# IuvenisSapiens/Qwen3-TTS-Rust

Measured on AMD Instinct MI355X. Metric: audio-seconds generated per second (aggregate over GPUs) = concurrent real-time streams; RTF and first-chunk latency from the single-utterance leg, higher is better.
Workload: dtype i8

## Files before the change

### qwen3-tts-rust_amd/csrc/kernels.hip

```cpp
#include "kernels.h"
#include <cstdlib>
#include "q3_common.h"
#include "../../include/q3tts_spec.h"
#include "kdev.h"
#include "wslice.h"

namespace q3 {

Q3_STAMP_SETTER(set_stamp_buffer)

template <int LPR, int MT>
__global__ void __launch_bounds__(512) k_gemv_q8(Q8Mat w, int row0, int nrows, const int8_t* __restrict__ xq,
                                                 const uint16_t* __restrict__ xd, float* __restrict__ out,
                                                 int out_stride, int ntok) {
    constexpr int R = 64 / LPR, BPL = LPR / 2, NLD = 8 / BPL;
    __shared__ float red[8][R * MT];
    const int lane = threadIdx.x & 63, wave = threadIdx.x >> 6;
    const int r = lane % R, q = lane / R, half = q & 1, bil = q >> 1;
    const int nseg = w.K >> 8, nb = w.K >> 5;
    const int sseg = blockIdx.y, seg = sseg * 8 + wave;
    const int tok0 = blockIdx.z * MT;
    const bool active = seg < nseg;
    float acc[MT];
#pragma unroll
    for (int m = 0; m < MT; m++) acc[m] = 0.0f;
    if (active) {
        int row = row0 + blockIdx.x * R + r;
        if (row > w.Npad - 1) row = w.Npad - 1;
        const int rg = row >> 5, r32 = row & 31;
        const uint8_t* base = w.qs + ((size_t)rg * nb + (size_t)seg * 8) * 1024 + half * 512 + r32 * 16;
        uint4 wv[NLD];
#pragma unroll
        for (int i = 0; i < NLD; i++) wv[i] = *reinterpret_cast<const uint4*>(base + (size_t)(i * BPL + bil) * 1024);
        const uint4 dwv = *reinterpret_cast<const uint4*>(w.sc + (((size_t)rg * nseg + seg) * 32 + r32) * 8);
#pragma unroll
        for (int m = 0; m < MT; m++) {
            int tok = tok0 + m;
            if (tok > ntok - 1) tok = ntok - 1;
            const int8_t* xp = xq + (size_t)tok * w.K + seg * 256;
            const uint4 dxv = *reinterpret_cast<const uint4*>(xd + (size_t)tok * nb + seg * 8);
#pragma unroll
            for (int i = 0; i < NLD; i++) {
                const uint4 xv = *reinterpret_cast<const uint4*>(xp + (i * BPL + bil) * 32 + half * 16);
                int isum = dot16(wv[i], xv);
                isum += xor_lane<R>(isum);
#pragma unroll
                for (int j = 0; j < BPL; j++) {
                    const int isj = (BPL == 1) ? isum : __shfl(isum, r + 2 * j * R);
                    const int b = i * BPL + j;
                    const float sc = h2f(half_of(dwv, b)) * h2f(half_of(dxv, b));
                    acc[m] = q3_fmaf((float)isj, sc, acc[m]);
                }
            }
        }
        if (q == 0) {
#pragma unroll
            for (int m = 0; m < MT; m++) red[wave][m * R + r] = acc[m];
        }
    }
    wg_barrier_lds();
    for (int t = threadIdx.x; t < R * MT; t += blockDim.x) {
        const int m = t / R, rr = t % R;
        int nsg = nseg - sseg * 8;
        if (nsg > 8) nsg = 8;
        float v[8];
#pragma unroll
        for (int s = 0; s < 8; s++) v[s] = red[s][t];
        float S = v[0];
#pragma unroll
        for (int s = 1; s < 8; s++) S = (s < nsg) ? S + v[s] : S;
        const int orow = blockIdx.x * R + rr, tok = tok0 + m;
        if (orow < nrows && tok < ntok) out[((size_t)sseg * ntok + tok) * out_stride + orow] = S;
    }
}

__global__ void k_gemm_q8_tok(Q8Mat w, int row0, int nrows, const int8_t* __restrict__ xq, const uint16_t* __restrict__ xd,
                              float* __restrict__ out, int out_stride, int ntok);
#define Q3_GEMM_Q8_BUDGET __launch_bounds__(512) __attribute__((amdgpu_waves_per_eu(4, 4)))
template <bool GU>
__global__ void Q3_GEMM_Q8_BUDGET k_gemm_q8_mfma(Q8Mat w, int row0, int nrows, const int8_t* __restrict__ xq, const uint16_t* __restrict__ xd,
                               float* __restrict__ out, int out_stride, int ntok, int ff, int8_t* __restrict__ aq, uint16_t* __restrict__ ad);
template <bool GU>
__global__ void Q3_GEMM_Q8_BUDGET k_gemm_q8_tile1(Q8Mat w, int row0, int nrows, const int8_t* __restrict__ xq, const uint16_t* __restrict__ xd,
                               float* __restrict__ out, int out_stride, int ntok, int ff, int8_t* __restrict__ aq, uint16_t* __restrict__ ad);
#define Q3_GEMM_Q8_WIDE_BUDGET __launch_bounds__(256) __attribute__((amdgpu_waves_per_eu(2, 2)))
template <bool GU>
__global__ void Q3_GEMM_Q8_WIDE_BUDGET k_gemm_q8_wide(Q8Mat w, int row0, int nrows, const int8_t* __restrict__ xq, const uint16_t* __restrict__ xd,
// ... 865 lines not shown
                        const int orow = blockIdx.x * 32 + rr;
                        if (orow < nrows && tok < ntok) out[((size_t)sseg * ntok + tok) * out_stride + orow] = S;
                    } else if (q == 0) gate_s[lt][t] = S;
                    else {
                        const float y = q3_swiglu(gate_s[lt][t], S);
                        float amax = q3_fabsf(y);
                        amax = fmaxf(amax, xor_lane<16>(amax)); amax = fmaxf(amax, xor_lane<8>(amax)); amax = fmaxf(amax, xor_lane<4>(amax));
                        amax = fmaxf(amax, xor_lane<2>(amax)); amax = fmaxf(amax, xor_lane<1>(amax));
                        const float dd = amax / 127.0f;
                        const float id = (dd != 0.0f) ? (1.0f / dd) : 0.0f;
                        if (tok < ntok) {
                            aq[(size_t)tok * ff + blockIdx.x * 32 + rr] = (int8_t)(int)q3_rintf(y * id);
                            if (rr == 0) ad[(size_t)tok * (ff >> 5) + blockIdx.x] = f2h(dd);
                        }
                    }
                }
                wg_barrier_lds();
            }
        }
    });
}


__global__ void __launch_bounds__(64) k_rmsnorm_quant(NormArgs a) {
    const int tok = blockIdx.x, lane = threadIdx.x;
    const int nch = a.d >> 8;
    const float* hin = a.h_in;
    if (a.idx_keys) hin += (size_t)key_code(a.idx_keys[(size_t)tok * a.idx_stride]) * a.h_stride;
    else if (a.idx) hin += (size_t)a.idx[(size_t)tok * a.idx_stride] * a.h_stride;
    else hin += (size_t)tok * a.h_stride;
    float4 x[8];
    float p = 0.0f;
#pragma unroll
    for (int c = 0; c < 8; c++) {
        if (c < nch) {
            float4 v = *reinterpret_cast<const float4*>(hin + 256 * c + 4 * lane);
            if (a.nparts > 0) {
                const float* pp = a.parts + (size_t)tok * a.parts_stride + 256 * c + 4 * lane;
                float4 y = *reinterpret_cast<const float4*>(pp);
                for (int s = 1; s < a.nparts; s++) {
                    const float4 z = *reinterpret_cast<const float4*>(pp + (size_t)s * gridDim.x * a.parts_stride);
                    y.x = y.x + z.x; y.y = y.y + z.y; y.z = y.z + z.z; y.w = y.w + z.w;
                }
                v.x = v.x + y.x; v.y = v.y + y.y; v.z = v.z + y.z; v.w = v.w + y.w;
            }
            if (a.h_out) *reinterpret_cast<float4*>(a.h_out + (size_t)tok * a.d + 256 * c + 4 * lane) = v;
            x[c] = v;
            p = q3_fmaf(v.x, v.x, p); p = q3_fmaf(v.y, v.y, p); p = q3_fmaf(v.z, v.z, p); p = q3_fmaf(v.w, v.w, p);
        }
    }
    const float ss = wave_sum_bfly(p);
    const float mean = ss / (float)a.d;
    const float scale = 1.0f / q3_sqrtf(mean + a.eps);
#pragma unroll
    for (int c = 0; c < 8; c++) {
        if (c < nch) {
            const float4 g = *reinterpret_cast<const float4*>(a.g + 256 * c + 4 * lane);
            float4 y;
            y.x = (x[c].x * scale) * g.x; y.y = (x[c].y * scale) * g.y;
            y.z = (x[c].z * scale) * g.z; y.w = (x[c].w * scale) * g.w;
            if (a.xn_out) *reinterpret_cast<float4*>(a.xn_out + (size_t)tok * a.d + 256 * c + 4 * lane) = y;
            float amax = fmaxf(fmaxf(q3_fabsf(y.x), q3_fabsf(y.y)), fmaxf(q3_fabsf(y.z), q3_fabsf(y.w)));
            amax = fmaxf(amax, xor_lane<1>(amax)); amax = fmaxf(amax, xor_lane<2>(amax)); amax = fmaxf(amax, xor_lane<4>(amax));
            const float dd = amax / 127.0f;
            const float id = (dd != 0.0f) ? (1.0f / dd) : 0.0f;
            const int q0 = (int)q3_rintf(y.x * id), q1 = (int)q3_rintf(y.y * id), q2 = (int)q3_rintf(y.z * id), q3v = (int)q3_rintf(y.w * id);
            const uint32_t pk = (uint32_t)(q0 & 0xFF) | ((uint32_t)(q1 & 0xFF) << 8) | ((uint32_t)(q2 & 0xFF) << 16) | ((uint32_t)(q3v & 0xFF) << 24);
            *reinterpret_cast<uint32_t*>(a.xq + (size_t)tok * a.d + 256 * c + 4 * lane) = pk;
            if ((lane & 7) == 0) a.xd[(size_t)tok * (a.d >> 5) + 8 * c + (lane >> 3)] = f2h(dd);
        }
    }
}
void launch_rmsnorm_quant(hipStream_t st, const NormArgs& a, int ntok) {
    hipLaunchKernelGGL(k_rmsnorm_quant, dim3(ntok), dim3(64), 0, st, a);
}

__global__ void __launch_bounds__(64) k_qk_rope_append(QkvRows qkv, int n_head, int n_kv,
                                                       const float* __restrict__ q_norm_w, const float* __restrict__ k_norm_w,
                                                       float eps, const float* __restrict__ rope_cos,
                                                       const float* __restrict__ rope_sin, int n_ctx,
                                                       const int32_t* __restrict__ mrope_sec, TokMeta tm, KvCache kv,
                                                       int layer, float* __restrict__ qrot) {
    const int hv = blockIdx.x, tok = blockIdx.y, lane = threadIdx.x;
    const float* vec = qkv.row(tok) + (size_t)hv * 128;
    float x1 = vec[lane], x2 = vec[lane + 64];
    const int seq = tm.seq_of(tok), slot = tm.slot_of(tok);
    const int page = kv.page_of(seq, slot >> 6);
    const int ps = slot & 63;
    if (hv < n_head + n_kv) {
        const float* w = hv < n_head ? q_norm_w : k_norm_w;
        float p = x1 * x1;
        p = q3_fmaf(x2, x2, p);
        const float ss = wave_sum_bfly(p);
        const float mean = ss / 128.0f;
        const float scale = 1.0f / q3_sqrtf(mean + eps);
        const float y1 = (x1 * scale) * w[lane], y2 = (x2 * scale) * w[lane + 64];
        int32_t sec[4] = { mrope_sec[0], mrope_sec[1], mrope_sec[2], mrope_sec[3] };
        int pp = tm.pos_of(tok, q3_mrope_stream(lane, sec));
        if (pp < 0) pp = 0;
        if (pp > n_ctx - 1) pp = n_ctx - 1;
        float o1, o2;
        q3_rope_pair(y1, y2, rope_cos[(size_t)pp * 64 + lane], rope_sin[(size_t)pp * 64 + lane], &o1, &o2);
        if (hv < n_head) {
            float* dst = qrot + ((size_t)tok * n_head + hv) * 128;
            dst[lane] = o1; dst[lane + 64] = o2;
        } else {
            const int kh = hv - n_head;
            uint16_t* Kb = kv.k + (size_t)page * kv.page_stride() + (size_t)layer * kv.layer_stride() + (size_t)kh * 8192;
            Kb[((lane >> 3) * 64 + ps) * 8 + (lane & 7)] = f2h(o1);
            Kb[(((lane + 64) >> 3) * 64 + ps) * 8 + (lane & 7)] = f2h(o2);
        }
    } else {
        const int vh = hv - n_head - n_kv;
        uint16_t* Vb = kv.v + (size_t)page * kv.page_stride() + (size_t)layer * kv.layer_stride() + (size_t)vh * 8192;
        Vb[ps * 128 + lane] = f2h(x1);
        Vb[ps * 128 + lane + 64] = f2h(x2);
    }
}
void launch_qk_rope_append(hipStream_t st, const QkvRows& qkv, const float*, int n_head, int n_kv,
                           const float* q_norm_w, const float* k_norm_w, float eps, const float* rope_cos,
                           const float* rope_sin, int n_ctx, const int32_t* mrope_sec, const TokMeta& tm,
                           const KvCache& kv, int layer, float* qrot, int ntok) {
    hipLaunchKernelGGL(k_qk_rope_append, dim3(n_head + 2 * n_kv, ntok), dim3(64), 0, st, qkv, n_head, n_kv,
                       q_norm_w, k_norm_w, eps, rope_cos, rope_sin, n_ctx, mrope_sec, tm, kv, layer, qrot);
}

__global__ void __launch_bounds__(256) __attribute__((amdgpu_waves_per_eu(4, 4)))
k_attention(const float* __restrict__ qrot, int n_head, int n_kv, TokMeta tm, KvCache kv, int layer, float* __restrict__ att,
            int8_t* __restrict__ aq, uint16_t* __restrict__ ad) {
    __shared__ __attribute__((aligned(16))) float q_s[128];
    __shared__ float p_s[256];
    __shared__ float red_s[4][128];
    __shared__ float wmax_s[4];
    const int tok = blockIdx.y, tid = threadIdx.x, lane = tid & 63, wave = __builtin_amdgcn_readfirstlane(tid >> 6);
    const int grp = n_head / n_kv, bx = blockIdx.x;
    const int h = (n_kv & 7) == 0 ? (bx % n_kv) * grp + bx / n_kv : bx;
    const int seq = tm.seq_of(tok), n = tm.slot_of(tok) + 1;
    const int kvh = h / grp;
    const size_t head_off = (size_t)layer * kv.layer_stride() + (size_t)kvh * 8192;
    const int jj = lane >> 4, dc = lane & 15;
    typedef const int32_t __attribute__((address_space(4))) * const_i32_ptr;
    const const_i32_ptr ptab = (const_i32_ptr)(uintptr_t)kv.page_table;
    auto page_of = [&](int logical) { return kv.page_table ? ptab[(size_t)seq * kv.max_pages + logical] : seq; };
    const float qv = qrot[((size_t)tok * n_head + h) * 128 + (tid & 127)];
    const float scale = 0.08838834764831845f;
    float M = 0.0f, L = 0.0f, O[8];
#pragma unroll
    for (int i = 0; i < 8; i++) O[i] = 0.0f;
    for (int c0 = 0; c0 < n; c0 += 256) {
        const int cn = (n - c0) < 256 ? (n - c0) : 256;
        const int jbase = c0 + wave * 64;
        float S[8], mc;
        auto chunk = [&](auto nb_const) {
            constexpr int NB = decltype(nb_const)::value;
            uint4 vreg[4 * NB];
            int pg[NB];
#pragma unroll
            for (int b = 0; b < NB; b++) pg[b] = page_of((c0 >> 6) + b);
            auto load_v = [&](int b, const float* after) {
                const uint16_t* Vb = kv.v + (size_t)pg[b] * kv.page_stride() + head_off;
#pragma unroll
                for (int g = 0; g < 4; g++) {
                    const int jg = c0 + 64 * b + 16 * g + 4 * wave + jj;
                    uint32_t off = (uint32_t)(((jg < n ? jg : n - 1) & 63) * 128 + dc * 8);
                    if (after) asm volatile("" : "+v"(off) : "v"(*after));
                    vreg[4 * b + g] = *reinterpret_cast<const uint4*>(Vb + off);
                }
            };
            auto q_handoff = [&]() {
                if (c0 == 0) {
                    q_s[tid & 127] = qv;
                    wg_barrier_lds();
                }
            };
            const bool valid = (jbase + lane) < n;
            float s = -INFINITY;
            if (jbase < n) {
                int pgk = pg[0];
#pragma unroll
                for (int b = 1; b < NB; b++) pgk = wave == b ? pg[b] : pgk;
                const uint16_t* Kb = kv.k + (size_t)pgk * kv.page_stride() + head_off;
                uint4 kreg[16];
#pragma unroll
                for (int d8 = 0; d8 < 16; d8++) kreg[d8] = *reinterpret_cast<const uint4*>(Kb + (d8 * 64 + lane) * 8);
                load_v(0, nullptr);
// ... 651 lines not shown
```

### qwen3-tts-rust_amd/csrc/kernels_fused.hip

```cpp
#include "kernels.h"
#include "kdev.h"
#include "wslice.h"
#include <cstdlib>
#include "q3_common.h"

namespace q3 {
Q3_STAMP_SETTER(set_stamp_buffer_fused)

__device__ __forceinline__ void norm_quant_token(const NormPro& a, int d, int tok, int ntok, int lane, int8_t* xq_dst,
                                                 uint16_t* xd_dst, bool write_global) {
    const int nch = d >> 8;
    const float* hin = a.h_in;
    if (a.idx_keys) hin += (size_t)key_code(a.idx_keys[(size_t)tok * a.idx_stride]) * a.h_stride;
    else hin += (size_t)tok * a.h_stride;
    float4 x[8];
    float p = 0.0f;
#pragma unroll
    for (int c = 0; c < 8; c++) {
        if (c < nch) {
            float4 v = *reinterpret_cast<const float4*>(hin + 256 * c + 4 * lane);
            if (a.nparts > 0) {
                const float* pp = a.parts + (size_t)tok * a.parts_stride + 256 * c + 4 * lane;
                float4 y = *reinterpret_cast<const float4*>(pp);
                for (int s = 1; s < a.nparts; s++) {
                    const float4 z = *reinterpret_cast<const float4*>(pp + (size_t)s * a.parts_slab);
                    y.x = y.x + z.x; y.y = y.y + z.y; y.z = y.z + z.z; y.w = y.w + z.w;
                }
                v.x = v.x + y.x; v.y = v.y + y.y; v.z = v.z + y.z; v.w = v.w + y.w;
            }
            if (write_global && a.h_out) *reinterpret_cast<float4*>(a.h_out + (size_t)tok * d + 256 * c + 4 * lane) = v;
            x[c] = v;
            p = q3_fmaf(v.x, v.x, p); p = q3_fmaf(v.y, v.y, p); p = q3_fmaf(v.z, v.z, p); p = q3_fmaf(v.w, v.w, p);
        }
    }
    const float ss = wave_sum_bfly(p);
    const float mean = ss / (float)d;
    const float scale = 1.0f / q3_sqrtf(mean + a.eps);
#pragma unroll
    for (int c = 0; c < 8; c++) {
        if (c < nch) {
            const float4 g = *reinterpret_cast<const float4*>(a.g + 256 * c + 4 * lane);
            float4 y;
            y.x = (x[c].x * scale) * g.x; y.y = (x[c].y * scale) * g.y;
            y.z = (x[c].z * scale) * g.z; y.w = (x[c].w * scale) * g.w;
            if (write_global && a.xn_out) *reinterpret_cast<float4*>(a.xn_out + (size_t)tok * d + 256 * c + 4 * lane) = y;
            float amax = fmaxf(fmaxf(q3_fabsf(y.x), q3_fabsf(y.y)), fmaxf(q3_fabsf(y.z), q3_fabsf(y.w)));
            amax = fmaxf(amax, xor_lane<1>(amax)); amax = fmaxf(amax, xor_lane<2>(amax)); amax = fmaxf(amax, xor_lane<4>(amax));
            const float dd = amax / 127.0f;
            const float id = (dd != 0.0f) ? (1.0f / dd) : 0.0f;
            const int q0 = (int)q3_rintf(y.x * id), q1 = (int)q3_rintf(y.y * id), q2 = (int)q3_rintf(y.z * id), q3v = (int)q3_rintf(y.w * id);
            const uint32_t pk = (uint32_t)(q0 & 0xFF) | ((uint32_t)(q1 & 0xFF) << 8) | ((uint32_t)(q2 & 0xFF) << 16) | ((uint32_t)(q3v & 0xFF) << 24);
            *reinterpret_cast<uint32_t*>(xq_dst + 256 * c + 4 * lane) = pk;
            if ((lane & 7) == 0) xd_dst[8 * c + (lane >> 3)] = f2h(dd);
        }
    }
}

__device__ __forceinline__ void norm_quant_wg(const NormPro& a, int d, int tok, bool tok_valid, int lane, int wave, int8_t* xq_dst,
                                              uint16_t* xd_dst, float* vbuf, float* scal, bool write_global) {
    const int c = wave;
    float4 v = make_float4(0.f, 0.f, 0.f, 0.f), g = v;
    if (tok_valid) {
        const float* hin = a.h_in;
        if (a.idx_keys) hin += (size_t)key_code(a.idx_keys[(size_t)tok * a.idx_stride]) * a.h_stride;
        else hin += (size_t)tok * a.h_stride;
        v = *reinterpret_cast<const float4*>(hin + 256 * c + 4 * lane);
        g = *reinterpret_cast<const float4*>(a.g + 256 * c + 4 * lane);
        if (a.nparts > 0) {
            const float* pp = a.parts + (size_t)tok * a.parts_stride + 256 * c + 4 * lane;
            float4 z[4];
            const int np = a.nparts < 4 ? a.nparts : 4;
#pragma unroll
            for (int s = 0; s < 4; s++) if (s < np) z[s] = *reinterpret_cast<const float4*>(pp + (size_t)s * a.parts_slab);
            float4 y = z[0];
#pragma unroll
            for (int s = 1; s < 4; s++) if (s < np) { y.x = y.x + z[s].x; y.y = y.y + z[s].y; y.z = y.z + z[s].z; y.w = y.w + z[s].w; }
            for (int s = 4; s < a.nparts; s++) {
                const float4 zz = *reinterpret_cast<const float4*>(pp + (size_t)s * a.parts_slab);
                y.x = y.x + zz.x; y.y = y.y + zz.y; y.z = y.z + zz.z; y.w = y.w + zz.w;
            }
            v.x = v.x + y.x; v.y = v.y + y.y; v.z = v.z + y.z; v.w = v.w + y.w;
        }
        if (write_global && a.h_out) *reinterpret_cast<float4*>(a.h_out + (size_t)tok * d + 256 * c + 4 * lane) = v;
    }
    *reinterpret_cast<float4*>(vbuf + 256 * c + 4 * lane) = v;
    wg_barrier_lds();
// ... 364 lines not shown
        const float mc = fmaxf(fmaxf(wmax_s[0], wmax_s[1]), fmaxf(wmax_s[2], wmax_s[3]));
        const float p = valid ? q3_expf(s - mc) : 0.0f;
        p_s[wave * 64 + lane] = p;
        wg_barrier_lds();
        float S[8];
#pragma unroll
        for (int i = 0; i < 8; i++) S[i] = 0.0f;
        const int cn = (n - c0) < 256 ? (n - c0) : 256;
#pragma unroll
        for (int u = 0; u < 16; u++) {
            if (16 * u < cn) {
                const int jl = 16 * u + 4 * wave + jj;
                const int jg = c0 + jl;
                const float pj = p_s[jl];
                uint4 vv = vreg[u];
                if (jg == slot) vv = *reinterpret_cast<const uint4*>(&vcur_s[dc * 8]);
                S[0] = q3_fmaf(pj, h2f(vv.x & 0xFFFFu), S[0]); S[1] = q3_fmaf(pj, h2f(vv.x >> 16), S[1]);
                S[2] = q3_fmaf(pj, h2f(vv.y & 0xFFFFu), S[2]); S[3] = q3_fmaf(pj, h2f(vv.y >> 16), S[3]);
                S[4] = q3_fmaf(pj, h2f(vv.z & 0xFFFFu), S[4]); S[5] = q3_fmaf(pj, h2f(vv.z >> 16), S[5]);
                S[6] = q3_fmaf(pj, h2f(vv.w & 0xFFFFu), S[6]); S[7] = q3_fmaf(pj, h2f(vv.w >> 16), S[7]);
            }
        }
#pragma unroll
        for (int i = 0; i < 8; i++) {
            const float a2 = S[i] + xor_lane<16>(S[i]);
            const float T = a2 + xor_lane<32>(a2);
            if (jj == 0) red_s[wave][dc * 8 + i] = T;
        }
        wg_barrier_lds();
        if (wave == 0) {
            float a2 = p_s[lane];
            a2 = a2 + p_s[lane + 64]; a2 = a2 + p_s[lane + 128]; a2 = a2 + p_s[lane + 192];
            const float lc = wave_sum_bfly(a2);
            float oc[8];
#pragma unroll
            for (int i = 0; i < 8; i++) oc[i] = (red_s[0][dc * 8 + i] + red_s[1][dc * 8 + i]) + (red_s[2][dc * 8 + i] + red_s[3][dc * 8 + i]);
            if (c0 == 0) {
                M = mc; L = lc;
#pragma unroll
                for (int i = 0; i < 8; i++) O[i] = oc[i];
            } else {
                const float mn = fmaxf(M, mc);
                const float ea = q3_expf(M - mn), eb = q3_expf(mc - mn);
                const float t2 = lc * eb;
                L = q3_fmaf(L, ea, t2);
#pragma unroll
                for (int i = 0; i < 8; i++) { const float u2 = oc[i] * eb; O[i] = q3_fmaf(O[i], ea, u2); }
                M = mn;
            }
        }
        wg_barrier_lds();
    }
    if (wave == 0) {
        float y[8];
        float amax = 0.0f;
#pragma unroll
        for (int i = 0; i < 8; i++) { y[i] = O[i] / L; amax = fmaxf(amax, q3_fabsf(y[i])); }
        amax = fmaxf(amax, xor_lane<1>(amax));
        amax = fmaxf(amax, xor_lane<2>(amax));
        const float dd = amax / 127.0f;
        const float id = (dd != 0.0f) ? (1.0f / dd) : 0.0f;
        if (jj == 0) {
            const size_t o = ((size_t)tok * n_head + h) * 128 + dc * 8;
            uint32_t lo = 0, hi = 0;
#pragma unroll
            for (int i = 0; i < 4; i++) {
                lo |= (uint32_t)((int)q3_rintf(y[i] * id) & 0xFF) << (8 * i);
                hi |= (uint32_t)((int)q3_rintf(y[i + 4] * id) & 0xFF) << (8 * i);
            }
            *reinterpret_cast<uint2*>(aq + o) = make_uint2(lo, hi);
            if ((dc & 3) == 0) ad[o >> 5] = f2h(dd);
        }
    }
}
void launch_attention_fused(hipStream_t st, const QkvRows& qkv, int n_head, int n_kv, const float* q_norm_w,
                            const float* k_norm_w, float eps, const float* rope_cos, const float* rope_sin, int n_ctx,
                            const int32_t* mrope_sec, const TokMeta& tm, const KvCache& kv, int layer, int8_t* aq, uint16_t* ad,
                            int ntok) {
    hipLaunchKernelGGL(k_attention_fused, dim3(n_head, ntok), dim3(256), 0, st, qkv, n_head, n_kv, q_norm_w, k_norm_w,
                       eps, rope_cos, rope_sin, n_ctx, mrope_sec, tm, kv, layer, aq, ad);
}

template <int HPW>
__global__ void __launch_bounds__(64) k_attention_short(QkvRows qkv, int n_head, int n_kv,
                                                        const float* __restrict__ q_norm_w, const float* __restrict__ k_norm_w, float eps,
                                                        const float* __restrict__ rope_cos, const float* __restrict__ rope_sin, int n_ctx,
                                                        const int32_t* __restrict__ mrope_sec, TokMeta tm, KvCache kv, int layer,
                                                        int8_t* __restrict__ aq, uint16_t* __restrict__ ad, float* __restrict__ att) {
    __shared__ __attribute__((aligned(16))) float q_s[HPW][128];
    __shared__ __attribute__((aligned(16))) uint16_t kcur_s[128];
    __shared__ __attribute__((aligned(16))) uint16_t vcur_s[128];
    __shared__ float p_s[HPW][64];
    const int kvh = HPW == 2 ? blockIdx.x : blockIdx.x >> 1, h0 = HPW == 2 ? 2 * blockIdx.x : blockIdx.x;
    Q3_STAMP_DECL;
    Q3_STAMP(0);
    const bool writer = HPW == 2 || (blockIdx.x & 1) == 0;
    const int tok = blockIdx.y, lane = threadIdx.x;
    const float* tv = qkv.row(tok);
    const float scale = 0.08838834764831845f;
    const int jj = lane >> 4, dc = lane & 15;
    const int seq = tm.seq_of(tok), slot = tm.slot_of(tok), n = slot + 1;
    const size_t head_off = (size_t)layer * kv.layer_stride() + (size_t)kvh * 8192;
    const int page = kv.page_of(seq, 0);
    const uint16_t* Kb = kv.k + (size_t)page * kv.page_stride() + head_off;
    const uint16_t* Vb = kv.v + (size_t)page * kv.page_stride() + head_off;
    uint4 kreg[16], vreg[4][4];
#pragma unroll
    for (int d8 = 0; d8 < 16; d8++) kreg[d8] = (lane < slot) ? *reinterpret_cast<const uint4*>(Kb + (d8 * 64 + lane) * 8) : make_uint4(0, 0, 0, 0);
#pragma unroll
    for (int ww = 0; ww < 4; ww++)
#pragma unroll
        for (int u = 0; u < 4; u++) {
            const int jl = 16 * u + 4 * ww + jj;
            vreg[ww][u] = (jl < slot) ? *reinterpret_cast<const uint4*>(Vb + jl * 128 + dc * 8) : make_uint4(0, 0, 0, 0);
        }
    int32_t sec[4] = { mrope_sec[0], mrope_sec[1], mrope_sec[2], mrope_sec[3] };
    int pp = tm.pos_of(tok, q3_mrope_stream(lane, sec));
    if (pp < 0) pp = 0;
    if (pp > n_ctx - 1) pp = n_ctx - 1;
    const float cs = rope_cos[(size_t)pp * 64 + lane], sn = rope_sin[(size_t)pp * 64 + lane];
#pragma unroll
    for (int which = 0; which < HPW + 1; which++) {
        const float* vec = tv + (which < HPW ? (size_t)(h0 + which) * 128 : (size_t)(n_head + kvh) * 128);
        const float* wn = which < HPW ? q_norm_w : k_norm_w;
        const float x1 = vec[lane], x2 = vec[lane + 64];
        float p = x1 * x1;
        p = q3_fmaf(x2, x2, p);
        const float ss = wave_sum_bfly(p);
        const float mean = ss / 128.0f;
        const float sc2 = 1.0f / q3_sqrtf(mean + eps);
        const float y1 = (x1 * sc2) * wn[lane], y2 = (x2 * sc2) * wn[lane + 64];
        float o1, o2;
        q3_rope_pair(y1, y2, cs, sn, &o1, &o2);
        if (which < HPW) { q_s[which][lane] = o1; q_s[which][lane + 64] = o2; }
        else {
            const uint16_t k1 = f2h(o1), k2 = f2h(o2);
            kcur_s[lane] = k1; kcur_s[lane + 64] = k2;
            if (writer) {
                uint16_t* Kw = kv.k + (size_t)page * kv.page_stride() + head_off;
                Kw[((lane >> 3) * 64 + slot) * 8 + (lane & 7)] = k1;
                Kw[(((lane + 64) >> 3) * 64 + slot) * 8 + (lane & 7)] = k2;
            }
        }
    }
    {
        const float* vec = tv + (size_t)(n_head + n_kv + kvh) * 128;
        const uint16_t v1 = f2h(vec[lane]), v2 = f2h(vec[lane + 64]);
        vcur_s[lane] = v1; vcur_s[lane + 64] = v2;
        if (writer) {
            uint16_t* Vw = kv.v + (size_t)page * kv.page_stride() + head_off;
            Vw[slot * 128 + lane] = v1; Vw[slot * 128 + lane + 64] = v2;
        }
    }
    wg_barrier_lds();
    Q3_STAMP(1);
    const bool valid = lane < n, cur = lane == slot;
    float a[HPW];
#pragma unroll
    for (int hh = 0; hh < HPW; hh++) a[hh] = 0.0f;
#pragma unroll
    for (int d8 = 0; d8 < 16; d8++) {
        uint4 kk = kreg[d8];
        if (cur) kk = *reinterpret_cast<const uint4*>(&kcur_s[8 * d8]);
        const float kf[8] = { h2f(kk.x & 0xFFFFu), h2f(kk.x >> 16), h2f(kk.y & 0xFFFFu), h2f(kk.y >> 16),
                              h2f(kk.z & 0xFFFFu), h2f(kk.z >> 16), h2f(kk.w & 0xFFFFu), h2f(kk.w >> 16) };
#pragma unroll
        for (int e = 0; e < 8; e++)
#pragma unroll
            for (int hh = 0; hh < HPW; hh++) a[hh] = q3_fmaf(q_s[hh][8 * d8 + e], kf[e], a[hh]);
    }
    Q3_STAMP_AFTER(2, a[0]);
    float L[HPW];
#pragma unroll
    for (int hh = 0; hh < HPW; hh++) {
        const float sc = valid ? a[hh] * scale : -INFINITY;
        const float m = wave_max_bfly(sc);
        const float pv = valid ? q3_expf(sc - m) : 0.0f;
        p_s[hh][lane] = pv;
        L[hh] = wave_sum_bfly(pv);
    }
    wg_barrier_lds();
    Q3_STAMP(3);
    const int dq = n_head * 128;
#pragma unroll
    for (int hh = 0; hh < HPW; hh++) {
        float s01[8], s23[8], y[8];
#pragma unroll
        for (int ww = 0; ww < 4; ww++) {
            float S[8];
#pragma unroll
            for (int i = 0; i < 8; i++) S[i] = 0.0f;
#pragma unroll
            for (int u = 0; u < 4; u++) {
                if (16 * u < n) {
                    const int jl = 16 * u + 4 * ww + jj;
                    const float pj = p_s[hh][jl];
                    uint4 vv = vreg[ww][u];
                    if (jl == slot) vv = *reinterpret_cast<const uint4*>(&vcur_s[dc * 8]);
                    S[0] = q3_fmaf(pj, h2f(vv.x & 0xFFFFu), S[0]); S[1] = q3_fmaf(pj, h2f(vv.x >> 16), S[1]);
                    S[2] = q3_fmaf(pj, h2f(vv.y & 0xFFFFu), S[2]); S[3] = q3_fmaf(pj, h2f(vv.y >> 16), S[3]);
                    S[4] = q3_fmaf(pj, h2f(vv.z & 0xFFFFu), S[4]); S[5] = q3_fmaf(pj, h2f(vv.z >> 16), S[5]);
                    S[6] = q3_fmaf(pj, h2f(vv.w & 0xFFFFu), S[6]); S[7] = q3_fmaf(pj, h2f(vv.w >> 16), S[7]);
                }
            }
#pragma unroll
            for (int i = 0; i < 8; i++) {
                const float a2 = S[i] + xor_lane<16>(S[i]);
                const float T = a2 + xor_lane<32>(a2);
                if (ww == 0) s01[i] = T; else if (ww == 1) s01[i] = s01[i] + T; else if (ww == 2) s23[i] = T; else s23[i] = s23[i] + T;
            }
        }
#pragma unroll
        for (int i = 0; i < 8; i++) y[i] = (s01[i] + s23[i]) / L[hh];
        const int hq = h0 + hh;
        if (att && jj == 0) {
            float* o = att + (size_t)tok * dq + (size_t)hq * 128 + dc * 8;
            *reinterpret_cast<float4*>(o) = make_float4(y[0], y[1], y[2], y[3]);
            *reinterpret_cast<float4*>(o + 4) = make_float4(y[4], y[5], y[6], y[7]);
        }
        float amax = 0.0f;
#pragma unroll
        for (int i = 0; i < 8; i++) amax = fmaxf(amax, q3_fabsf(y[i]));
        amax = fmaxf(amax, xor_lane<1>(amax));
        amax = fmaxf(amax, xor_lane<2>(amax));
        const float dd = amax / 127.0f;
        const float id = (dd != 0.0f) ? (1.0f / dd) : 0.0f;
        if (jj == 0) {
            uint32_t lo = 0, hi = 0;
#pragma unroll
            for (int i = 0; i < 4; i++) {
                lo |= (uint32_t)((int)q3_rintf(y[i] * id) & 0xFF) << (8 * i);
                hi |= (uint32_t)((int)q3_rintf(y[i + 4] * id) & 0xFF) << (8 * i);
            }
            *reinterpret_cast<uint2*>(aq + (size_t)tok * dq + (size_t)hq * 128 + dc * 8) = make_uint2(lo, hi);
            if ((dc & 3) == 0) ad[(size_t)tok * (dq >> 5) + hq * 4 + (dc >> 2)] = f2h(dd);
        }
    }
    Q3_STAMP(6);
    Q3_STAMP_FLUSH();
}
int short_attn_hpw1_max() {
    static const int v = [] { const char* e = std::getenv("Q3_SHORT_ATTN_HPW1_MAX"); return e ? atoi(e) : 128; }();
    return v;
}
void launch_attention_short(hipStream_t st, int hpw, const QkvRows& qkv, int n_head, int n_kv, const float* q_norm_w,
                            const float* k_norm_w, float eps, const float* rope_cos, const float* rope_sin, int n_ctx,
                            const int32_t* mrope_sec, const TokMeta& tm, const KvCache& kv, int layer, int8_t* aq, uint16_t* ad, int ntok, float* att) {
    if (hpw == 1)
        hipLaunchKernelGGL(k_attention_short<1>, dim3(n_head, ntok), dim3(64), 0, st, qkv, n_head, n_kv, q_norm_w, k_norm_w, eps, rope_cos,
                           rope_sin, n_ctx, mrope_sec, tm, kv, layer, aq, ad, att);
    else
        hipLaunchKernelGGL(k_attention_short<2>, dim3(n_kv, ntok), dim3(64), 0, st, qkv, n_head, n_kv, q_norm_w, k_norm_w, eps, rope_cos,
                           rope_sin, n_ctx, mrope_sec, tm, kv, layer, aq, ad, att);
}

__global__ void __launch_bounds__(256) k_project_mt(const float* __restrict__ x, int x_stride, const float* __restrict__ Wblk,
                                                    const float* __restrict__ b, int n_in, int n_out, float* __restrict__ out,
                                                    int out_stride, int ntok) {
    constexpr int KC = 512, LDP = KC + 4;
    __shared__ __attribute__((aligned(16))) float xs[16][LDP];
    __shared__ __attribute__((aligned(16))) float ws[16][LDP];
    const int ob = blockIdx.x, t0 = blockIdx.y * 16, tid = threadIdx.x;
    const int o16 = tid & 15, tl = tid >> 4;
    const float* wslab = Wblk + (size_t)ob * n_in * 16;
    float4 rx[8], rw[8];
    auto fetch = [&](int k0) {
#pragma unroll
        for (int j = 0; j < 8; j++) {
            const int e = tid + 256 * j;
            const int t = e >> 7, i4 = e & 127;
            rx[j] = (t0 + t < ntok) ? *reinterpret_cast<const float4*>(x + (size_t)(t0 + t) * x_stride + k0 + 4 * i4) : make_float4(0.f, 0.f, 0.f, 0.f);
            rw[j] = *reinterpret_cast<const float4*>(wslab + (size_t)k0 * 16 + 4 * (size_t)e);
        }
    };
    auto stash = [&]() {
#pragma unroll
        for (int j = 0; j < 8; j++) {
            const int e = tid + 256 * j;
            *reinterpret_cast<float4*>(&xs[e >> 7][4 * (e & 127)]) = rx[j];
            const int i = e >> 2, q = (e & 3) * 4;
            ws[q + 0][i] = rw[j].x; ws[q + 1][i] = rw[j].y; ws[q + 2][i] = rw[j].z; ws[q + 3][i] = rw[j].w;
        }
    };
    const int o = ob * 16 + o16;
    float sum = b[o];
    fetch(0);
    for (int k0 = 0; k0 < n_in; k0 += KC) {
        stash();
        __syncthreads();
        if (k0 + KC < n_in) fetch(k0 + KC);
#pragma unroll 8
        for (int i = 0; i < KC; i += 4) {
            const float4 xv = *reinterpret_cast<const float4*>(&xs[tl][i]), wv = *reinterpret_cast<const float4*>(&ws[o16][i]);
            float t = xv.x * wv.x; sum = sum + t;
            t = xv.y * wv.y; sum = sum + t;
            t = xv.z * wv.z; sum = sum + t;
            t = xv.w * wv.w; sum = sum + t;
        }
        __syncthreads();
    }
    if (t0 + tl < ntok) out[(size_t)(t0 + tl) * out_stride + o] = sum;
}
void init_fused_kernel_attributes() {}
void launch_project_blk(hipStream_t st, const float* x, int x_stride, const float* Wblk, const float* b, int n_in, int n_out,
                        float* out, int out_stride, int ntok) {
    if (n_in % 512 != 0 || x_stride % 4 != 0 || (reinterpret_cast<uintptr_t>(x) & 15) != 0) throw Error("k_project_mt: n_in must be a multiple of 512 and the rows 16-byte aligned");
    if (n_out % 16 != 0) throw Error("k_project_mt: n_out must be a multiple of 16");
    hipLaunchKernelGGL(k_project_mt, dim3(n_out / 16, (ntok + 15) / 16), dim3(256), 0, st, x, x_stride, Wblk, b, n_in, n_out, out, out_stride, ntok);
}

template <bool TRAIL>
__global__ void __launch_bounds__(256) k_feedback_keys(const float* const* __restrict__ tables, const int64_t* __restrict__ table_rows,
                                                       const u64* __restrict__ keys, int key_stride,
                                                       const float* __restrict__ tts_pad, float* __restrict__ out, TextTrail tt) {
    const int tok = blockIdx.y, i = blockIdx.x * 256 + threadIdx.x;
    float acc = 0.0f;
#pragma unroll
    for (int q = 0; q < 16; q++) {
        int c = key_code(keys[(size_t)tok * key_stride + q]);
        if (c < 0) c = 0;
        const float v = ((int64_t)c < table_rows[q]) ? tables[q][(size_t)c * 2048 + i] : 0.0f;
// ... 149 lines not shown
```

Before: 757.1.

## Restructure short attention front-end with scalar token metadata and slot-specialized load schedules

Adds a shared helper that reads per-token metadata (seq, slot, page, mrope positions) through the constant address space so it stays in scalar registers. The QK-rope-append and short-attention kernels hoist all global loads (qkv rows, norm weights, rope tables) ahead of the compute behind a scheduling barrier. Short attention is specialized on slot count (0, up to 16, more), skips K/V loads that are not needed, defers V loads until after the QK dot product, and double-buffers Q reads from LDS. It also fixes waves-per-EU occupancy. This adds code size and fragile compiler-steering asm, and a lazy V-load path for HPW=2.

```diff
diff --git a/qwen3-tts-rust_amd/csrc/attn_front.h b/qwen3-tts-rust_amd/csrc/attn_front.h
--- /dev/null
+++ b/qwen3-tts-rust_amd/csrc/attn_front.h
@@ -0,0 +1,51 @@
+#pragma once
+#include "kernels.h"
+#include "kdev.h"
+
+namespace q3 {
+
+typedef const int32_t __attribute__((address_space(4))) * const_i32_ptr;
+typedef const unsigned long long __attribute__((address_space(4))) * const_u64_ptr;
+
+struct TokFront {
+    int seq, slot, page;
+    int pp[4];
+    int32_t sec[4];
+    const float* row;
+    __device__ __forceinline__ int pos_of_lane(int lane) const {
+        const int s = q3_mrope_stream(lane, sec);
+        return s == 0 ? pp[0] : s == 1 ? pp[1] : s == 2 ? pp[2] : pp[3];
+    }
+};
+
+__device__ __forceinline__ TokFront tok_front(const QkvRows& qkv, const int32_t* mrope_sec, const TokMeta& tm, const KvCache& kv, int n_ctx, int tok) {
+    TokFront f;
+    const const_i32_ptr csec = (const_i32_ptr)(uintptr_t)mrope_sec;
+#pragma unroll
+    for (int i = 0; i < 4; i++) f.sec[i] = csec[i];
+    int rowi = tok;
+    if (qkv.keys) rowi = (int)(~(uint32_t)((const_u64_ptr)(uintptr_t)qkv.keys)[(size_t)tok * qkv.key_stride]);
+    if (tm.uniform_pos >= 0) {
+        f.seq = tok; f.slot = tm.uniform_pos;
+#pragma unroll
+        for (int i = 0; i < 4; i++) f.pp[i] = tm.uniform_pos;
+    } else {
+        f.seq = ((const_i32_ptr)(uintptr_t)tm.seq)[tok];
+        f.slot = ((const_i32_ptr)(uintptr_t)tm.slot)[tok];
+        const const_i32_ptr cpos = (const_i32_ptr)(uintptr_t)tm.pos;
+#pragma unroll
+        for (int i = 0; i < 4; i++) f.pp[i] = cpos[(size_t)tok * 4 + i];
+    }
+    f.page = kv.page_table ? ((const_i32_ptr)(uintptr_t)kv.page_table)[(size_t)f.seq * kv.max_pages + (f.slot >> 6)] : f.seq;
+#pragma unroll
+    for (int i = 0; i < 4; i++) {
+        if (f.pp[i] < 0) f.pp[i] = 0;
+        if (f.pp[i] > n_ctx - 1) f.pp[i] = n_ctx - 1;
+    }
+    f.row = qkv.base + (size_t)rowi * qkv.stride;
+    asm volatile("" :: "s"(f.seq), "s"(f.slot), "s"(f.page), "s"(f.pp[0]), "s"(f.pp[1]), "s"(f.pp[2]), "s"(f.pp[3]), "s"(f.sec[0]), "s"(f.sec[1]),
+                 "s"(f.sec[2]), "s"(f.sec[3]), "s"(f.row));
+    return f;
+}
+
+}
diff --git a/qwen3-tts-rust_amd/csrc/kernels.hip b/qwen3-tts-rust_amd/csrc/kernels.hip
--- a/qwen3-tts-rust_amd/csrc/kernels.hip
+++ b/qwen3-tts-rust_amd/csrc/kernels.hip
@@ -3,6 +3,7 @@
 #include "q3_common.h"
 #include "../../include/q3tts_spec.h"
 #include "kdev.h"
+#include "attn_front.h"
 #include "wslice.h"
 
 namespace q3 {
@@ -1034,25 +1035,27 @@
                                                        const int32_t* __restrict__ mrope_sec, TokMeta tm, KvCache kv,
                                                        int layer, float* __restrict__ qrot) {
     const int hv = blockIdx.x, tok = blockIdx.y, lane = threadIdx.x;
-    const float* vec = qkv.row(tok) + (size_t)hv * 128;
-    float x1 = vec[lane], x2 = vec[lane + 64];
-    const int seq = tm.seq_of(tok), slot = tm.slot_of(tok);
-    const int page = kv.page_of(seq, slot >> 6);
-    const int ps = slot & 63;
+    asm volatile("" :: "s"(qkv.base), "s"(qkv.keys), "s"(qkv.stride), "s"(qkv.key_stride), "s"(n_head), "s"(n_kv), "s"(q_norm_w), "s"(k_norm_w),
+                 "s"(eps), "s"(rope_cos), "s"(rope_sin), "s"(n_ctx), "s"(mrope_sec), "s"(tm.seq), "s"(tm.slot), "s"(tm.pos), "s"(tm.uniform_pos),
+                 "s"(kv.k), "s"(kv.v), "s"(kv.page_table), "s"(kv.max_pages), "s"(kv.n_layer), "s"(kv.n_kv), "s"(layer), "s"(qrot));
+    const TokFront f = tok_front(qkv, mrope_sec, tm, kv, n_ctx, tok);
+    const float* vec = f.row + (size_t)hv * 128;
+    const int page = f.page, ps = f.slot & 63;
+    const float* w = hv < n_head ? q_norm_w : k_norm_w;
+    const int pp = f.pos_of_lane(lane);
+    const float x1 = vec[lane], x2 = vec[lane + 64], w1 = w[lane], w2 = w[lane + 64];
+    const float cs = rope_cos[(size_t)pp * 64 + lane], sn = rope_sin[(size_t)pp * 64 + lane];
+    asm volatile("" ::: "memory");
+    __builtin_amdgcn_sched_barrier(0);
     if (hv < n_head + n_kv) {
-        const float* w = hv < n_head ? q_norm_w : k_norm_w;
         float p = x1 * x1;
         p = q3_fmaf(x2, x2, p);
         const float ss = wave_sum_bfly(p);
         const float mean = ss / 128.0f;
         const float scale = 1.0f / q3_sqrtf(mean + eps);
-        const float y1 = (x1 * scale) * w[lane], y2 = (x2 * scale) * w[lane + 64];
-        int32_t sec[4] = { mrope_sec[0], mrope_sec[1], mrope_sec[2], mrope_sec[3] };
-        int pp = tm.pos_of(tok, q3_mrope_stream(lane, sec));
-        if (pp < 0) pp = 0;
-        if (pp > n_ctx - 1) pp = n_ctx - 1;
+        const float y1 = (x1 * scale) * w1, y2 = (x2 * scale) * w2;
         float o1, o2;
-        q3_rope_pair(y1, y2, rope_cos[(size_t)pp * 64 + lane], rope_sin[(size_t)pp * 64 + lane], &o1, &o2);
+        q3_rope_pair(y1, y2, cs, sn, &o1, &o2);
         if (hv < n_head) {
             float* dst = qrot + ((size_t)tok * n_head + hv) * 128;
             dst[lane] = o1; dst[lane + 64] = o2;
diff --git a/qwen3-tts-rust_amd/csrc/kernels_fused.hip b/qwen3-tts-rust_amd/csrc/kernels_fused.hip
--- a/qwen3-tts-rust_amd/csrc/kernels_fused.hip
+++ b/qwen3-tts-rust_amd/csrc/kernels_fused.hip
@@ -1,7 +1,9 @@
 #include "kernels.h"
 #include "kdev.h"
+#include "attn_front.h"
 #include "wslice.h"
 #include <cstdlib>
+#include <type_traits>
 #include "q3_common.h"
 
 namespace q3 {
@@ -532,7 +534,7 @@
 }
 
 template <int HPW>
-__global__ void __launch_bounds__(64) k_attention_short(QkvRows qkv, int n_head, int n_kv,
+__global__ void __launch_bounds__(64) __attribute__((amdgpu_waves_per_eu(4, 4))) k_attention_short(QkvRows qkv, int n_head, int n_kv,
                                                         const float* __restrict__ q_norm_w, const float* __restrict__ k_norm_w, float eps,
                                                         const float* __restrict__ rope_cos, const float* __restrict__ rope_sin, int n_ctx,
                                                         const int32_t* __restrict__ mrope_sec, TokMeta tm, KvCache kv, int layer,
@@ -541,45 +543,74 @@
     __shared__ __attribute__((aligned(16))) uint16_t kcur_s[128];
     __shared__ __attribute__((aligned(16))) uint16_t vcur_s[128];
     __shared__ float p_s[HPW][64];
+    __shared__ float l_s[HPW];
     const int kvh = HPW == 2 ? blockIdx.x : blockIdx.x >> 1, h0 = HPW == 2 ? 2 * blockIdx.x : blockIdx.x;
     Q3_STAMP_DECL;
     Q3_STAMP(0);
     const bool writer = HPW == 2 || (blockIdx.x & 1) == 0;
     const int tok = blockIdx.y, lane = threadIdx.x;
-    const float* tv = qkv.row(tok);
+    asm volatile("" :: "s"(qkv.base), "s"(qkv.keys), "s"(qkv.stride), "s"(qkv.key_stride), "s"(n_head), "s"(n_kv), "s"(q_norm_w), "s"(k_norm_w),
+                 "s"(eps), "s"(rope_cos), "s"(rope_sin), "s"(n_ctx), "s"(mrope_sec), "s"(tm.seq), "s"(tm.slot), "s"(tm.pos), "s"(tm.uniform_pos),
+                 "s"(kv.k), "s"(kv.v), "s"(kv.page_table), "s"(kv.max_pages), "s"(kv.n_layer), "s"(kv.n_kv), "s"(layer), "s"(aq), "s"(ad), "s"(att));
+    const TokFront f = tok_front(qkv, mrope_sec, tm, kv, n_ctx, tok);
     const float scale = 0.08838834764831845f;
     const int jj = lane >> 4, dc = lane & 15;
-    const int seq = tm.seq_of(tok), slot = tm.slot_of(tok), n = slot + 1;
+    const int slot = f.slot, n = slot + 1;
     const size_t head_off = (size_t)layer * kv.layer_stride() + (size_t)kvh * 8192;
-    const int page = kv.page_of(seq, 0);
-    const uint16_t* Kb = kv.k + (size_t)page * kv.page_stride() + head_off;
-    const uint16_t* Vb = kv.v + (size_t)page * kv.page_stride() + head_off;
+    const uint16_t* Kb = kv.k + (size_t)f.page * kv.page_stride() + head_off;
+    const uint16_t* Vb = kv.v + (size_t)f.page * kv.page_stride() + head_off;
+    auto body = [&](auto nu_const) {
+    constexpr int NU = decltype(nu_const)::value;
+    constexpr int NUP = HPW == 1 ? 1 : 0;
+    constexpr bool LAZY = HPW == 2 && NU == 4;
+    constexpr int NUR = NU == 0 ? 1 : NU == 1 ? 2 : 4;
+    asm volatile("; instance %0" :: "n"(NU) : "memory");
+    int ln = lane;
+    asm volatile("" : "+v"(ln));
+    float xr[HPW + 2][2];
+#pragma unroll
+    for (int which = 0; which < HPW + 2; which++) {
+        const float* vec = f.row + (which < HPW ? (size_t)(h0 + which) * 128 : which == HPW ? (size_t)(n_head + kvh) * 128 : (size_t)(n_head + n_kv + kvh) * 128);
+        xr[which][0] = vec[ln]; xr[which][1] = vec[ln + 64];
+    }
+    const float wq1 = q_norm_w[ln], wq2 = q_norm_w[ln + 64], wk1 = k_norm_w[ln], wk2 = k_norm_w[ln + 64];
+    const int pp = f.pos_of_lane(lane);
+    const float cs = rope_cos[(size_t)pp * 64 + ln], sn = rope_sin[(size_t)pp * 64 + ln];
+    asm volatile("" ::: "memory");
     uint4 kreg[16], vreg[4][4];
 #pragma unroll
-    for (int d8 = 0; d8 < 16; d8++) kreg[d8] = (lane < slot) ? *reinterpret_cast<const uint4*>(Kb + (d8 * 64 + lane) * 8) : make_uint4(0, 0, 0, 0);
+    for (int d8 = 0; d8 < 16; d8++) kreg[d8] = make_uint4(0, 0, 0, 0);
 #pragma unroll
     for (int ww = 0; ww < 4; ww++)
 #pragma unroll
-        for (int u = 0; u < 4; u++) {
+        for (int u = 0; u < 4; u++) vreg[ww][u] = make_uint4(0, 0, 0, 0);
+    const int last = slot - 1;
+    auto load_v = [&](int u, const float* after) {
+#pragma unroll
+        for (int ww = 0; ww < 4; ww++) {
             const int jl = 16 * u + 4 * ww + jj;
-            vreg[ww][u] = (jl < slot) ? *reinterpret_cast<const uint4*>(Vb + jl * 128 + dc * 8) : make_uint4(0, 0, 0, 0);
-        }
-    int32_t sec[4] = { mrope_sec[0], mrope_sec[1], mrope_sec[2], mrope_sec[3] };
-    int pp = tm.pos_of(tok, q3_mrope_stream(lane, sec));
-    if (pp < 0) pp = 0;
-    if (pp > n_ctx - 1) pp = n_ctx - 1;
-    const float cs = rope_cos[(size_t)pp * 64 + lane], sn = rope_sin[(size_t)pp * 64 + lane];
+            uint32_t off = (uint32_t)((jl < last ? jl : last) * 128 + dc * 8);
+            if (after) asm volatile("" : "+v"(off) : "v"(*after));
+            vreg[ww][u] = *reinterpret_cast<const uint4*>(Vb + off);
+        }
+    };
+    if (NU > 0) {
+        const int kl = lane < last ? lane : last;
+#pragma unroll
+        for (int d8 = 0; d8 < 16; d8++) kreg[d8] = *reinterpret_cast<const uint4*>(Kb + (d8 * 64 + kl) * 8);
+        if (NUP > 0) load_v(0, nullptr);
+    }
+    asm volatile("" ::: "memory");
+    __builtin_amdgcn_sched_barrier(0);
 #pragma unroll
     for (int which = 0; which < HPW + 1; which++) {
-        const float* vec = tv + (which < HPW ? (size_t)(h0 + which) * 128 : (size_t)(n_head + kvh) * 128);
-        const float* wn = which < HPW ? q_norm_w : k_norm_w;
-        const float x1 = vec[lane], x2 = vec[lane + 64];
+        const float x1 = xr[which][0], x2 = xr[which][1];
         float p = x1 * x1;
         p = q3_fmaf(x2, x2, p);
         const float ss = wave_sum_bfly(p);
         const float mean = ss / 128.0f;
         const float sc2 = 1.0f / q3_sqrtf(mean + eps);
-        const float y1 = (x1 * sc2) * wn[lane], y2 = (x2 * sc2) * wn[lane + 64];
+        const float y1 = (x1 * sc2) * (which < HPW ? wq1 : wk1), y2 = (x2 * sc2) * (which < HPW ? wq2 : wk2);
         float o1, o2;
         q3_rope_pair(y1, y2, cs, sn, &o1, &o2);
         if (which < HPW) { q_s[which][lane] = o1; q_s[which][lane + 64] = o2; }
@@ -587,18 +618,17 @@
             const uint16_t k1 = f2h(o1), k2 = f2h(o2);
             kcur_s[lane] = k1; kcur_s[lane + 64] = k2;
             if (writer) {
-                uint16_t* Kw = kv.k + (size_t)page * kv.page_stride() + head_off;
+                uint16_t* Kw = kv.k + (size_t)f.page * kv.page_stride() + head_off;
                 Kw[((lane >> 3) * 64 + slot) * 8 + (lane & 7)] = k1;
                 Kw[(((lane + 64) >> 3) * 64 + slot) * 8 + (lane & 7)] = k2;
             }
         }
     }
     {
-        const float* vec = tv + (size_t)(n_head + n_kv + kvh) * 128;
-        const uint16_t v1 = f2h(vec[lane]), v2 = f2h(vec[lane + 64]);
+        const uint16_t v1 = f2h(xr[HPW + 1][0]), v2 = f2h(xr[HPW + 1][1]);
         vcur_s[lane] = v1; vcur_s[lane + 64] = v2;
         if (writer) {
-            uint16_t* Vw = kv.v + (size_t)page * kv.page_stride() + head_off;
+            uint16_t* Vw = kv.v + (size_t)f.page * kv.page_stride() + head_off;
             Vw[slot * 128 + lane] = v1; Vw[slot * 128 + lane + 64] = v2;
         }
     }
@@ -608,18 +638,42 @@
     float a[HPW];
 #pragma unroll
     for (int hh = 0; hh < HPW; hh++) a[hh] = 0.0f;
+    float qf[HPW][8];
+#pragma unroll
+    for (int hh = 0; hh < HPW; hh++) {
+        const float4 qa = *reinterpret_cast<const float4*>(&q_s[hh][0]), qb = *reinterpret_cast<const float4*>(&q_s[hh][4]);
+        qf[hh][0] = qa.x; qf[hh][1] = qa.y; qf[hh][2] = qa.z; qf[hh][3] = qa.w; qf[hh][4] = qb.x; qf[hh][5] = qb.y; qf[hh][6] = qb.z; qf[hh][7] = qb.w;
+    }
 #pragma unroll
     for (int d8 = 0; d8 < 16; d8++) {
         uint4 kk = kreg[d8];
         if (cur) kk = *reinterpret_cast<const uint4*>(&kcur_s[8 * d8]);
         const float kf[8] = { h2f(kk.x & 0xFFFFu), h2f(kk.x >> 16), h2f(kk.y & 0xFFFFu), h2f(kk.y >> 16),
                               h2f(kk.z & 0xFFFFu), h2f(kk.z >> 16), h2f(kk.w & 0xFFFFu), h2f(kk.w >> 16) };
+        float nf[HPW][8];
+        if (d8 < 15) {
+            int qi = 8 * (d8 + 1);
+            asm volatile("" : "+v"(qi) : "v"(a[HPW - 1]));
+#pragma unroll
+            for (int hh = 0; hh < HPW; hh++) {
+                const float4 qa = *reinterpret_cast<const float4*>(&q_s[hh][qi]), qb = *reinterpret_cast<const float4*>(&q_s[hh][qi + 4]);
+                nf[hh][0] = qa.x; nf[hh][1] = qa.y; nf[hh][2] = qa.z; nf[hh][3] = qa.w; nf[hh][4] = qb.x; nf[hh][5] = qb.y; nf[hh][6] = qb.z; nf[hh][7] = qb.w;
+            }
+        }
 #pragma unroll
         for (int e = 0; e < 8; e++)
 #pragma unroll
-            for (int hh = 0; hh < HPW; hh++) a[hh] = q3_fmaf(q_s[hh][8 * d8 + e], kf[e], a[hh]);
+            for (int hh = 0; hh < HPW; hh++) a[hh] = q3_fmaf(qf[hh][e], kf[e], a[hh]);
+        if (d8 < 15) {
+#pragma unroll
+            for (int hh = 0; hh < HPW; hh++)
+#pragma unroll
+                for (int e = 0; e < 8; e++) qf[hh][e] = nf[hh][e];
+        }
     }
     Q3_STAMP_AFTER(2, a[0]);
+#pragma unroll
+    for (int u = NUP; u < (LAZY ? 0 : NU); u++) load_v(u, &a[0]);
     float L[HPW];
 #pragma unroll
     for (int hh = 0; hh < HPW; hh++) {
@@ -628,6 +682,7 @@
         const float pv = valid ? q3_expf(sc - m) : 0.0f;
         p_s[hh][lane] = pv;
         L[hh] = wave_sum_bfly(pv);
+        if (LAZY) l_s[hh] = L[hh];
     }
     wg_barrier_lds();
     Q3_STAMP(3);
@@ -641,12 +696,15 @@
 #pragma unroll
             for (int i = 0; i < 8; i++) S[i] = 0.0f;
 #pragma unroll
-            for (int u = 0; u < 4; u++) {
+            for (int u = 0; u < NUR; u++) {
                 if (16 * u < n) {
                     const int jl = 16 * u + 4 * ww + jj;
                     const float pj = p_s[hh][jl];
                     uint4 vv = vreg[ww][u];
+                    if (LAZY) vv = *reinterpret_cast<const uint4*>(Vb + (jl < last ? jl : last) * 128 + dc * 8);
+                    if (!(jl < slot)) vv = make_uint4(0, 0, 0, 0);
                     if (jl == slot) vv = *reinterpret_cast<const uint4*>(&vcur_s[dc * 8]);
+                    if (HPW > 1) asm volatile("" : "+v"(vv.x), "+v"(vv.y), "+v"(vv.z), "+v"(vv.w));
                     S[0] = q3_fmaf(pj, h2f(vv.x & 0xFFFFu), S[0]); S[1] = q3_fmaf(pj, h2f(vv.x >> 16), S[1]);
                     S[2] = q3_fmaf(pj, h2f(vv.y & 0xFFFFu), S[2]); S[3] = q3_fmaf(pj, h2f(vv.y >> 16), S[3]);
                     S[4] = q3_fmaf(pj, h2f(vv.z & 0xFFFFu), S[4]); S[5] = q3_fmaf(pj, h2f(vv.z >> 16), S[5]);
@@ -661,10 +719,12 @@
             }
         }
 #pragma unroll
-        for (int i = 0; i < 8; i++) y[i] = (s01[i] + s23[i]) / L[hh];
+        for (int i = 0; i < 8; i++) y[i] = (s01[i] + s23[i]) / (LAZY ? l_s[hh] : L[hh]);
         const int hq = h0 + hh;
+        int dce = dc;
+        if (LAZY) asm volatile("" : "+v"(dce) : "v"(y[0]));
         if (att && jj == 0) {
-            float* o = att + (size_t)tok * dq + (size_t)hq * 128 + dc * 8;
+            float* o = att + (size_t)tok * dq + (size_t)hq * 128 + dce * 8;
             *reinterpret_cast<float4*>(o) = make_float4(y[0], y[1], y[2], y[3]);
             *reinterpret_cast<float4*>(o + 4) = make_float4(y[4], y[5], y[6], y[7]);
         }
@@ -682,11 +742,15 @@
                 lo |= (uint32_t)((int)q3_rintf(y[i] * id) & 0xFF) << (8 * i);
                 hi |= (uint32_t)((int)q3_rintf(y[i + 4] * id) & 0xFF) << (8 * i);
             }
-            *reinterpret_cast<uint2*>(aq + (size_t)tok * dq + (size_t)hq * 128 + dc * 8) = make_uint2(lo, hi);
-            if ((dc & 3) == 0) ad[(size_t)tok * (dq >> 5) + hq * 4 + (dc >> 2)] = f2h(dd);
+            *reinterpret_cast<uint2*>(aq + (size_t)tok * dq + (size_t)hq * 128 + dce * 8) = make_uint2(lo, hi);
+            if ((dce & 3) == 0) ad[(size_t)tok * (dq >> 5) + hq * 4 + (dce >> 2)] = f2h(dd);
         }
     }
     Q3_STAMP(6);
+    };
+    if (slot == 0) body(std::integral_constant<int, 0>());
+    else if (slot <= 16) body(std::integral_constant<int, 1>());
+    else body(std::integral_constant<int, 4>());
     Q3_STAMP_FLUSH();
 }
 int short_attn_hpw1_max() {
```

Measured after the change: 624.4. 17.5% lower.
